# OthmanB/TAMCMC-C-

Measured on AMD Instinct MI355X. Metric: MALA steps/sec (all chains) + achieved HBM GB/s, 64 chains × 1e5-bin spectrum, higher is better.
Workload: dtype f64; 1 GPU; C2: model_MS_Global_a1etaa3_HarveyLike (id 2), 21 modes l=0..2, 56 params, 100000 bins, 64 chains per GPU, trunc_c=20, logL + gradient over 44 variables, params resident in HBM; chains_total=64

## Files before the change

tamcmc-c-_amd/csrc/tamcmc_eval_body.h:

```cpp
#ifndef TAMCMC_EVAL_BODY_H
#define TAMCMC_EVAL_BODY_H
#include <hip/hip_runtime.h>
#include "tamcmc_dev.h"

#define TM_WAVES (TM_THREADS / 64)

typedef const __attribute__((address_space(4))) TmMult *TmMultK;
typedef const __attribute__((address_space(4))) TmCellRec *TmCellRecK;
typedef const __attribute__((address_space(4))) TmTileHdr *TmTileHdrK;
typedef const __attribute__((address_space(4))) TmNoise *TmNoiseK;
typedef const __attribute__((address_space(4))) int32_t *TmIdxK;
typedef const __attribute__((address_space(4))) TmActive *TmActiveK;

typedef int TmEntry __attribute__((ext_vector_type(4)));
__device__ __forceinline__ TmEntry tm_load_entry(TmActiveK p)
{
    return *reinterpret_cast<const __attribute__((address_space(4))) TmEntry *>(p);
}

__device__ __forceinline__ double tm_rcp(double x)
{
    double r = __builtin_amdgcn_rcp(x);
    double e = __builtin_fma(-x, r, 1.0);
    r = __builtin_fma(r, e, r);
    e = __builtin_fma(-x, r, 1.0);
    r = __builtin_fma(r, e, r);
    return r;
}

__device__ __forceinline__ double tm_rcp1(double x)
{
    double r = __builtin_amdgcn_rcp(x);
    const double e = __builtin_fma(-x, r, 1.0);
    return __builtin_fma(r, e, r);
}

template <int MASK>
__device__ __forceinline__ unsigned tm_xor_dw(unsigned v, int lane)
{
    if constexpr (MASK == 1) return __builtin_amdgcn_update_dpp(0u, v, 0xB1, 0xf, 0xf, false);
    else if constexpr (MASK == 2) return __builtin_amdgcn_update_dpp(0u, v, 0x4E, 0xf, 0xf, false);
    else if constexpr (MASK == 4) {
        const unsigned r = __builtin_amdgcn_update_dpp(0u, v, 0x104, 0xf, 0x5, false);
        return __builtin_amdgcn_update_dpp(r, v, 0x114, 0xf, 0xa, false);
    } else if constexpr (MASK == 8) return __builtin_amdgcn_update_dpp(0u, v, 0x128, 0xf, 0xf, false);
    else if constexpr (MASK == 16) {
        const auto r = __builtin_amdgcn_permlane16_swap(v, v, false, false);
        return (lane & 16) ? r[0] : r[1];
    } else {
        const auto r = __builtin_amdgcn_permlane32_swap(v, v, false, false);
        return (lane & 32) ? r[0] : r[1];
    }
}

template <int MASK>
__device__ __forceinline__ double tm_xor(double v, int lane)
{
    const unsigned long long b = __double_as_longlong(v);
    const unsigned lo = tm_xor_dw<MASK>((unsigned)b, lane), hi = tm_xor_dw<MASK>((unsigned)(b >> 32), lane);
    return __longlong_as_double(((unsigned long long)hi << 32) | lo);
}

template <int MASK>
__device__ __forceinline__ double tm_swap_add(double a, double b)
{
    static_assert(MASK == 16 || MASK == 32, "two-register swaps exist for 16 and 32 lanes");
    const unsigned long long ba = __double_as_longlong(a), bb = __double_as_longlong(b);
    unsigned r0l, r1l, r0h, r1h;
    if constexpr (MASK == 32) {
        const auto l = __builtin_amdgcn_permlane32_swap((unsigned)ba, (unsigned)bb, false, false);
        const auto h = __builtin_amdgcn_permlane32_swap((unsigned)(ba >> 32), (unsigned)(bb >> 32), false, false);
        r0l = l[0]; r1l = l[1]; r0h = h[0]; r1h = h[1];
    } else {
        const auto l = __builtin_amdgcn_permlane16_swap((unsigned)ba, (unsigned)bb, false, false);
        const auto h = __builtin_amdgcn_permlane16_swap((unsigned)(ba >> 32), (unsigned)(bb >> 32), false, false);
        r0l = l[0]; r1l = l[1]; r0h = h[0]; r1h = h[1];
    }
    const double r0 = __longlong_as_double(((unsigned long long)r0h << 32) | r0l);
    const double r1 = __longlong_as_double(((unsigned long long)r1h << 32) | r1l);
    return r0 + r1;
}

__device__ __forceinline__ double tm_wave_sum(double v)
{
    const int lane = threadIdx.x & 63;
    v += tm_xor<32>(v, lane);
    v += tm_xor<16>(v, lane);
    v += tm_xor<8>(v, lane);
    v += tm_xor<4>(v, lane);
    v += tm_xor<2>(v, lane);
    v += tm_xor<1>(v, lane);
    return v;
}

__device__ __forceinline__ double tm_wave_prod(double v)
{
    const int lane = threadIdx.x & 63;
    v *= tm_xor<32>(v, lane);
    v *= tm_xor<16>(v, lane);
    v *= tm_xor<8>(v, lane);
    v *= tm_xor<4>(v, lane);
    v *= tm_xor<2>(v, lane);
    v *= tm_xor<1>(v, lane);
    return v;
}


__device__ __forceinline__ double tm_poly(TmCellRecK tr, double z)
{
    double p = tr->bg[TM_PDEG];
#pragma unroll
    for (int j = TM_PDEG - 1; j >= 0; j--) p = __builtin_fma(p, z, tr->bg[j]);
    return p;
}

template <int N, int MASK>
struct TmBfly {
    static constexpr int NE = (N + 1) & ~1;
    static constexpr int H = NE / 2;
    __device__ static __forceinline__ void run(double (&v)[TM_GSLOTS], int lane)
    {
        if constexpr (N == 1) {
            v[0] += tm_xor<MASK>(v[0], lane);
        } else if constexpr (MASK >= 16) {
#pragma unroll
            for (int i = 0; i < H; i++) v[i] = tm_swap_add<MASK>(v[i], (i + H < N) ? v[i + H] : 0.0);
        } else {
            const bool hi = (lane & MASK) != 0;
#pragma unroll
            for (int i = 0; i < H; i++) {
                const double up = (i + H < N) ? v[i + H] : 0.0;
                const double send = hi ? v[i] : up;
                const double keep = hi ? up : v[i];
                v[i] = keep + tm_xor<MASK>(send, lane);
            }
        }
        if constexpr (MASK > 1) TmBfly<(N == 1 ? 1 : H), MASK / 2>::run(v, lane);
    }
    __device__ static __forceinline__ int slot_of(int lane, bool &valid)
    {
        if constexpr (N == 1) {
            return 0;
        } else {
            int sub = 0;
            if constexpr (MASK > 1) sub = TmBfly<H, MASK / 2>::slot_of(lane, valid);
            const int idx = sub + (((lane & MASK) != 0) ? H : 0);
            if (idx >= N) valid = false;
            return idx;
        }
    }
};

template <int NC>
__device__ __forceinline__ double tm_mult_value(double x2, const double (&nu2)[NC], const double (&hq)[NC], double g2,
                                                double (&d)[NC], double (&r)[NC])
{
    double E[NC], P[NC];
#pragma unroll
    for (int m = 0; m < NC; m++) {
        d[m] = x2 - nu2[m];
        E[m] = __builtin_fma(d[m], d[m], g2);
    }
    P[0] = E[0];
#pragma unroll
    for (int m = 1; m < NC; m++) P[m] = P[m - 1] * E[m];
    double inv = tm_rcp1(P[NC - 1]);
    double s = 0.0;
#pragma unroll
    for (int m = NC - 1; m >= 1; m--) {
        r[m] = inv * P[m - 1];
        inv = inv * E[m];
    }
    r[0] = inv;
#pragma unroll
    for (int m = 0; m < NC; m++) s = __builtin_fma(hq[m], r[m], s);
    return s;
}

template <int NC>
__device__ __forceinline__ double tm_mult_sum(double x2, const double (&nu2)[NC], const double (&hq)[NC], double g2)
{
    double d = x2 - nu2[0];
    double Q = __builtin_fma(d, d, g2);
    double N = hq[0];
#pragma unroll
    for (int m = 1; m < NC; m++) {
        d = x2 - nu2[m];
        const double E = __builtin_fma(d, d, g2);
        N = __builtin_fma(hq[m], Q, N * E);
        Q = Q * E;
    }
    return N * tm_rcp(Q);
}

template <int NC, int KG, bool ASYM>
__device__ __forceinline__ void tm_accum_mult(TmMultK sm, const double (&x2)[KG], const int (&bi)[KG], double (&acc)[KG], const bool edge)
{
    double nu2[NC], hq[NC];
#pragma unroll
    for (int m = 0; m < NC; m++) { nu2[m] = sm->nu2[m]; hq[m] = sm->hq[m]; }
    const double g2 = sm->g2;
    const double aAh = ASYM ? 0.5 * sm->aA : 0.0, aB = ASYM ? sm->aB : 1.0, c2 = ASYM ? sm->c2 : 0.0;
    double s[KG];
#pragma unroll
    for (int k = 0; k < KG; k++) {
        s[k] = tm_mult_sum<NC>(x2[k], nu2, hq, g2);
        if (ASYM) {
            const double a = __builtin_fma(x2[k], aAh, aB);
            s[k] = s[k] * __builtin_fma(a, a, c2);
        }
    }
    if (edge) {
        const int imin = sm->imin, imax = sm->imax;
#pragma unroll
        for (int k = 0; k < KG; k++) {
            const bool inside = (bi[k] >= imin) && (bi[k] < imax);
            s[k] = inside ? s[k] : 0.0;
        }
    }
#pragma unroll
    for (int k = 0; k < KG; k++) acc[k] += s[k];
}

template <int KG>
__device__ __forceinline__ void tm_accum_dispatch(TmMultK sm, const int shape, const double (&x2)[KG], const int (&bi)[KG], double (&acc)[KG], const bool edge)
{
    switch (shape) {
    case 1: tm_accum_mult<1, KG, false>(sm, x2, bi, acc, edge); break;
    case 3: tm_accum_mult<3, KG, false>(sm, x2, bi, acc, edge); break;
    case 5: tm_accum_mult<5, KG, false>(sm, x2, bi, acc, edge); break;
    case 7: tm_accum_mult<7, KG, false>(sm, x2, bi, acc, edge); break;
    case 256 + 1: tm_accum_mult<1, KG, true>(sm, x2, bi, acc, edge); break;
    case 256 + 3: tm_accum_mult<3, KG, true>(sm, x2, bi, acc, edge); break;
    case 256 + 5: tm_accum_mult<5, KG, true>(sm, x2, bi, acc, edge); break;
    default: tm_accum_mult<7, KG, true>(sm, x2, bi, acc, edge); break;
    }
}

template <int NC> struct TmGradSlots {
    static constexpr int L = (NC - 1) / 2;
    static constexpr int A0 = NC, C = NC + L + 1, ASYM0 = NC + L + 2;
    __device__ static constexpr int count(bool asym) { return asym ? ASYM0 + 3 : ASYM0; }
};
template <int NC> __device__ __forceinline__ int tm_grad_store_slot(int v)
{
    using SL = TmGradSlots<NC>;
    return (v < NC) ? v : (v < SL::C) ? 7 + (v - NC) : (v == SL::C) ? 11 : 21 + (v - SL::ASYM0);
}

template <int NC, bool ASYM>
__device__ __forceinline__ void tm_grad_bin(const double (&nu2)[NC], const double (&hq)[NC], double g2, double aAh, double aB, double c2,
                                            const double x2, const double wk, double (&g)[TM_GSLOTS])
{
    using SL = TmGradSlots<NC>;
    double d[NC], r[NC];
    const double Sv = tm_mult_value<NC>(x2, nu2, hq, g2, d, r);
    double wA = wk;
    if (ASYM) {
        const double a = __builtin_fma(x2, aAh, aB);
        wA = wk * __builtin_fma(a, a, c2);
        const double ws = wk * Sv;
        g[SL::ASYM0 + 0] += ws;
        g[SL::ASYM0 + 1] = __builtin_fma(ws, a, g[SL::ASYM0 + 1]);
        g[SL::ASYM0 + 2] = __builtin_fma(ws * a, 0.5 * x2, g[SL::ASYM0 + 2]);
    }
#pragma unroll
    for (int m = 0; m < NC; m++) {
        const double t1 = wA * r[m];
        const double t2 = t1 * r[m];
        const int am = (m >= SL::L) ? m - SL::L : SL::L - m;
        g[SL::A0 + am] += t1;
        g[m] = __builtin_fma(t2, d[m], g[m]);
        g[SL::C] = __builtin_fma(hq[m], t2, g[SL::C]);
    }
}

template <int NC, bool ASYM>
__device__ __forceinline__ void tm_grad_unit(const double (&nu2)[NC], const double (&hq)[NC], double g2, double aAh, double aB, double c2,
                                             int imin, int imax, const double *__restrict__ gx, const double *wq, int i0, int Nx,
                                             const bool edge, double (&g)[TM_GSLOTS])
{
#pragma unroll
    for (int k = 0; k < 2; k++) {
        double x2, wk;
        if (edge) {
            const int i = i0 + k * TM_THREADS;
            const bool inside = (i >= imin) && (i < imax) && (i < Nx);
            x2 = gx[i < Nx ? i : Nx - 1];
            wk = inside ? wq[k * TM_THREADS] : 0.0;
        } else {
            x2 = gx[i0 + k * TM_THREADS];
            wk = wq[k * TM_THREADS];
        }
        tm_grad_bin<NC, ASYM>(nu2, hq, g2, aAh, aB, c2, x2, wk, g);
    }
}

template <int NC, bool ASYM>
__device__ __forceinline__ void tm_grad_unit_held(const double (&nu2)[NC], const double (&hq)[NC], double g2, double aAh, double aB, double c2,
                                                  int imin, int imax, const double (&xv)[2], const double (&wv)[2], int lo, int tid, int Nx,
                                                  const bool edge, double (&g)[TM_GSLOTS])
{
    double wk[2] = {wv[0], wv[1]};
    if (edge) {
#pragma unroll
        for (int k = 0; k < 2; k++) {
            const int i = lo + tid + k * TM_THREADS;
            const bool inside = (i >= imin) && (i < imax) && (i < Nx);
            wk[k] = inside ? wk[k] : 0.0;
        }
        asm volatile("" : "+v"(wk[0]), "+v"(wk[1]));
    }
#pragma unroll
    for (int k = 0; k < 2; k++) tm_grad_bin<NC, ASYM>(nu2, hq, g2, aAh, aB, c2, xv[k], wk[k], g);
}

__device__ __forceinline__ void tm_grad_fetch(const double *__restrict__ gx, const double *s_w, int u, int u0, int Nx, int tid,
                                              double (&xv)[2], double (&wv)[2])
{
    const int lo = u << TM_UNIT_SHIFT;
    if (lo + TM_UNIT_BINS <= Nx) {
        typedef const __attribute__((address_space(1))) double *TmGlobalD;
        TmGlobalD xb = (TmGlobalD)(gx + lo);
        asm volatile("" : "+s"(xb));
#pragma unroll
        for (int k = 0; k < 2; k++) xv[k] = xb[(unsigned)(tid + k * TM_THREADS)];
    } else {
#pragma unroll
        for (int k = 0; k < 2; k++) { const int i = lo + tid + k * TM_THREADS; xv[k] = gx[i < Nx ? i : Nx - 1]; }
        asm volatile("");
    }
    const double *wq = s_w + (u - u0) * TM_UNIT_BINS + tid;
#pragma unroll
    for (int k = 0; k < 2; k++) wv[k] = wq[k * TM_THREADS];
}

template <int NC, bool ASYM, bool AHEAD_>
__device__ __forceinline__ void tm_grad_mult(TmMultK sm, const double *__restrict__ gx, const double *s_w,
                                             int u0, int u1, int Nx, int tid, int lane, double *s_red_row)
{
    constexpr bool AHEAD = AHEAD_ && NC < 7;
    constexpr int V = TmGradSlots<NC>::count(ASYM);
    double g[TM_GSLOTS];
    double nu2[NC], hq[NC];
#pragma unroll
    for (int m = 0; m < NC; m++) { nu2[m] = sm->nu2[m]; hq[m] = sm->hq[m]; }
    const double g2 = sm->g2;
    const int imin = sm->imin, imax = sm->imax;
    const double aAh = ASYM ? 0.5 * sm->aA : 0.0, aB = ASYM ? sm->aB : 1.0, c2 = ASYM ? sm->c2 : 0.0;
#pragma unroll
    for (int s = 0; s < TM_GSLOTS; s++) g[s] = 0.0;
    if constexpr (AHEAD) {
        int ua = imin >> TM_UNIT_SHIFT, ub = (imax + TM_UNIT_BINS - 1) >> TM_UNIT_SHIFT;
        ua = ua > u0 ? ua : u0;
        ub = ub < u1 ? ub : u1;
        if (ua < ub) {
            double xc[2], wc[2];
            tm_grad_fetch(gx, s_w, ua, u0, Nx, tid, xc, wc);
            asm volatile("" : "+v"(xc[0]), "+v"(xc[1]), "+v"(wc[0]), "+v"(wc[1]));
            double xd[2], wd[2];
#pragma unroll 1
            for (int u = ua;;) {
                tm_grad_fetch(gx, s_w, u + 1 < ub ? u + 1 : u, u0, Nx, tid, xd, wd);
                {
                    const int lo = u << TM_UNIT_SHIFT, hi = lo + TM_UNIT_BINS;
                    tm_grad_unit_held<NC, ASYM>(nu2, hq, g2, aAh, aB, c2, imin, imax, xc, wc, lo, tid, Nx, !(lo >= imin && hi <= imax && hi <= Nx), g);
                }
                if (++u >= ub) break;
                tm_grad_fetch(gx, s_w, u + 1 < ub ? u + 1 : u, u0, Nx, tid, xc, wc);
                {
                    const int lo = u << TM_UNIT_SHIFT, hi = lo + TM_UNIT_BINS;
                    tm_grad_unit_held<NC, ASYM>(nu2, hq, g2, aAh, aB, c2, imin, imax, xd, wd, lo, tid, Nx, !(lo >= imin && hi <= imax && hi <= Nx), g);
                }
                if (++u >= ub) break;
            }
        }
    } else {
#pragma unroll 1
        for (int u = u0; u < u1; u++) {
            const int lo = u << TM_UNIT_SHIFT, hi = lo + TM_UNIT_BINS;
            if (hi <= imin || lo >= imax) continue;
            const double *wq = s_w + (u - u0) * TM_UNIT_BINS + tid;
            tm_grad_unit<NC, ASYM>(nu2, hq, g2, aAh, aB, c2, imin, imax, gx, wq, lo + tid, Nx, !(lo >= imin && hi <= imax && hi <= Nx), g);
        }
    }
#if defined(TM_ABLATE) && (TM_ABLATE & 1)
    if (lane == 0) s_red_row[0] = g[0] + g[1] + g[2];
    return;
#endif
    if constexpr (AHEAD) asm volatile("" : "+v"(lane));
    TmBfly<V, 32>::run(g, lane);
    constexpr int NSPLIT = (V > 16) ? 5 : (V > 8) ? 4 : (V > 4) ? 3 : (V > 2) ? 2 : 1;
    const int lowmask = (64 >> NSPLIT) - 1;
    bool valid = true;
    const int slot = TmBfly<V, 32>::slot_of(lane, valid);
    if ((lane & lowmask) == 0 && valid) {
        s_red_row[tm_grad_store_slot<NC>(slot)] = g[0];
    }
}

#ifndef TM_LB_FWD
#define TM_LB_FWD 4
#endif
#ifndef TM_LB_GRAD
#define TM_LB_GRAD 4
#endif
#ifndef TM_LOOKAHEAD
#define TM_LOOKAHEAD 1
#endif
#ifdef TM_TRACE
__device__ unsigned long long *g_tm_trace = nullptr;
#define TM_STAMP(slot) do { if (threadIdx.x == 0 && g_tm_trace) g_tm_trace[((size_t)blockIdx.y * gridDim.x + blockIdx.x) * 4 + (slot)] = wall_clock64(); } while (0)
#else
#define TM_STAMP(slot) do { } while (0)
#endif

#pragma clang fp contract(off)
__device__ __forceinline__ double tm_add_plain(double a, double b) { return a + b; }
#pragma clang fp contract(fast)

template <int N> struct TmInt { static constexpr int value = N; };
template <bool B> struct TmBool { static constexpr bool value = B; };

enum TmCellKind { TM_CK_POLY = 0, TM_CK_EXP = 1, TM_CK_NONE = 2, TM_CK_ANY = 3 };

template <bool GRAD, bool GEN = true>
__device__ __forceinline__ void tm_eval_body(const TmEvalArgs &a, const int chain, const int tile, double *s_w)
{
    const int like = GEN ? a.likelihood_case : 0;
    const int tid = threadIdx.x;
    const int lane = tid & 63, wave = tid >> 6;
    TmNoiseK sn = (TmNoiseK)(a.noise + chain);

#if defined(TM_ABLATE) && (TM_ABLATE & 16)
    if (a.Nx > 0) return;
#endif
    __shared__ double s_red[2][TM_WAVES][TM_GSLOTS];

    const size_t spec_off = (a.spec != nullptr) ? (size_t)((TmIdxK)a.spec)[chain] * (size_t)a.Nx : 0;
    const double *__restrict__ yp = a.y + spec_off;
    const double *__restrict__ isp = a.isig2 + spec_off;
    const TmMult *__restrict__ gm = a.mult + (size_t)chain * a.n_mult;
    TmTileHdrK th = (TmTileHdrK)(a.thdr + (size_t)chain * a.tiles + tile);
    const int u0 = th->u0;
    int u1 = th->u1;
    if (u1 - u0 > (GRAD ? TM_TILE_MAXU : TM_TILE_MAXU_L)) u1 = u0 + (GRAD ? TM_TILE_MAXU : TM_TILE_MAXU_L);
    const int nact = th->nact;
    TmCellRecK cells = (TmCellRecK)(a.cell + (size_t)chain * a.cells);
    TmActiveK tix = (TmActiveK)(a.tidx + ((size_t)chain * a.tiles + tile) * (a.n_mult > 0 ? a.n_mult : 1));
    const int nh = sn->nh;
    const bool has_gauss = GEN && sn->has_gauss != 0;
    const double N0 = sn->N0;
    const int row = (GEN && a.row_of_chain != nullptr) ? a.row_of_chain[chain] : -1;
    const double *__restrict__ xb = a.x2;
    const double *__restrict__ lb = a.lx;

#if defined(TM_ABLATE) && (TM_ABLATE & 32)
    if (nact >= 0 && N0 == N0) { if (tid == 0 && !GRAD) a.part[((size_t)chain * a.tiles + tile) * 4] = (double)(nh + row + u0 + (has_gauss ? 1 : 0)); return; }
#endif
    double S1 = 0.0;
    double P = 1.0;
    int esum = 0;
    int sgn = 0;
    double gn_[GRAD ? TM_GSLOTS : 1];
#pragma unroll
    for (int s_ = 0; s_ < (GRAD ? TM_GSLOTS : 1); s_++) gn_[s_] = 0.0;
    const double wscale = GRAD ? a.wt[2 * chain + 1] : 0.0;

    auto group = [&](auto kg_c, auto full_c, auto kind_c, const int u, TmCellRecK tr) __attribute__((always_inline)) {
        constexpr int KG = decltype(kg_c)::value;
        constexpr bool FULL = decltype(full_c)::value;
        constexpr int CK = decltype(kind_c)::value & 7;
        constexpr bool COLD = (decltype(kind_c)::value & 8) != 0;
        constexpr bool RT = CK == TM_CK_ANY;
        const bool HARVEY = RT ? nh > 0 : CK != TM_CK_NONE;
        const bool NPOLY = RT ? (nh > 0 && tr->npoly != 0) : CK == TM_CK_POLY;
        const int lo = u << TM_UNIT_SHIFT, hi = lo + KG * TM_THREADS;
        int nhx = nh;
        if constexpr (COLD) asm volatile("" : "+s"(nhx));
        double x2[KG], acc[KG];
        int bi[KG];
#pragma unroll
        for (int k = 0; k < KG; k++) {
            const int i = lo + k * TM_THREADS + tid;
            if (FULL) {
                bi[k] = i;
                x2[k] = xb[(unsigned)i];
            } else {
                const bool valid = i < a.Nx;
                bi[k] = valid ? i : -1;
                x2[k] = a.x2[valid ? i : a.Nx - 1];
            }
            acc[k] = 0.0;
        }
        constexpr bool EARLY = FULL && !GRAD && !COLD;
        double lxe[EARLY ? KG : 1], ye[EARLY ? KG : 1];
        if constexpr (EARLY) {
#pragma unroll
            for (int k = 0; k < KG; k++) { lxe[k] = HARVEY ? lb[(unsigned)bi[k]] : 0.0; ye[k] = yp[(unsigned)bi[k]]; }
        }
        if constexpr (GRAD) {
            for (int jj = 0; jj < nact; jj++) {
                const int idx = tix[jj].idx, imin = tix[jj].imin, imax = tix[jj].imax, shape = tix[jj].shape;
                if (hi <= imin || lo >= imax) continue;
                tm_accum_dispatch<KG>((TmMultK)(gm + idx), shape, x2, bi, acc, !(FULL && lo >= imin && hi <= imax));
            }
        } else if (nact > 0) {
            TmEntry e = tm_load_entry(tix);
            asm volatile("" :: "s"(e.x));
            for (int jj = 0; jj < nact; jj++) {
                const TmEntry en = tm_load_entry(tix + (jj + 1 < nact ? jj + 1 : jj));
                const int idx = e.x, imin = e.y, imax = e.z, shape = e.w;
                if (!(hi <= imin || lo >= imax))
                    tm_accum_dispatch<KG>((TmMultK)(gm + idx), shape, x2, bi, acc, !(FULL && lo >= imin && hi <= imax));
                e = en;
            }
        }

        constexpr int KH = GRAD ? 2 : KG;
#pragma unroll
        for (int h0 = 0; h0 < KG; h0 += KH) {
        double hu[TM_MAXH][GRAD ? KH : 1], harg[GRAD ? KH : 1];
        const bool n0_done = NPOLY;
        if (HARVEY) {
            double dl[KH];
#pragma unroll
            for (int k = 0; k < KH; k++) {
#if defined(TM_ABLATE) && (TM_ABLATE & 128)
                dl[k] = tr->lxc + 1e-9 * x2[h0 + k];
#else
                dl[k] = EARLY ? lxe[h0 + k] : FULL ? lb[(unsigned)bi[h0 + k]] : a.lx[bi[h0 + k] >= 0 ? bi[h0 + k] : a.Nx - 1];
#endif
                if constexpr (GRAD) harg[k] = dl[k];
            }
            if (NPOLY) {
                const double lxc = tr->lxc;
#pragma unroll
                for (int k = 0; k < KH; k++) { dl[k] -= lxc; acc[h0 + k] += tm_poly(tr, dl[k]); if constexpr (GRAD) harg[k] = dl[k]; }
            } else {
#pragma unroll
                for (int h = 0; h < TM_MAXH; h++) {
                    if (h < nhx) {
                        const double Hh = sn->H[h], ph = sn->p[h], lth = sn->lt[h];
#pragma unroll
                        for (int k = 0; k < KH; k++) {
                            const double t = exp(ph * (lth + dl[k]));
                            const double uu = 1.0 / (t + 1.0);
                            acc[h0 + k] += Hh * uu;
                            if constexpr (GRAD) hu[h][k] = uu;
                        }
                    }
                }
            }
        }
        if (has_gauss) {
            const double gA = sn->gA, gnu0 = sn->gnu0, gs2 = sn->gs2;
#pragma unroll
            for (int k = 0; k < KH; k++) {
                const double dd = 0.5 * x2[h0 + k] - gnu0;
                acc[h0 + k] = gA * exp((-0.5 * (dd * dd)) / gs2) + acc[h0 + k];
            }
        }
        if (!n0_done) {
#pragma unroll
            for (int k = 0; k < KH; k++) acc[h0 + k] += N0;
        }
        if (row >= 0) {
#pragma unroll
            for (int k = 0; k < KH; k++)
                if (FULL || bi[h0 + k] >= 0) a.model_out[(size_t)row * a.Nx + (size_t)(lo + (h0 + k) * TM_THREADS + tid)] = acc[h0 + k];
        }

        double wreg[GRAD ? KH : 1];
        if (like == 0) {
#pragma unroll
            for (int k = 0; k < KH; k++) {
                double wv = 0.0;
                if (FULL || bi[h0 + k] >= 0) {
                    const double M = acc[h0 + k];
                    const double yv = EARLY ? ye[h0 + k] : FULL ? yp[(unsigned)bi[h0 + k]] : yp[bi[h0 + k]];
                    sgn |= __double2hiint(M);
                    const double rM = tm_rcp(M);
                    S1 = __builtin_fma(yv, rM, S1);
                    int e;
                    P *= frexp(M, &e);
                    esum += e;
                    wv = wscale * (yv * rM * rM - rM);
                }
                if constexpr (GRAD) wreg[k] = wv;
            }
            {
                int e;
                P = frexp(P, &e);
                esum += e;
            }
        } else {
#pragma unroll
            for (int k = 0; k < KH; k++) {
                double wv = 0.0;
                if (FULL || bi[h0 + k] >= 0) {
                    const int i = lo + (h0 + k) * TM_THREADS + tid;
                    const double dd = yp[i] - acc[h0 + k];
                    const double is2 = isp[i];
                    S1 = __builtin_fma(dd * dd, is2, S1);
                    wv = wscale * dd * is2;
                }
                if constexpr (GRAD) wreg[k] = wv;
            }
        }
        if constexpr (GRAD) {
#pragma unroll
            for (int k = 0; k < KH; k++) {
                const double wk = wreg[k];
                s_w[((u - u0) * 2 + h0 + k) * TM_THREADS + tid] = wk;
                gn_[3 * TM_MAXH] = tm_add_plain(gn_[3 * TM_MAXH], wk);
#if defined(TM_ABLATE) && (TM_ABLATE & 512)
                if (false) {
#else
                if (NPOLY) {
#endif
                    double q = wk;
#pragma unroll
                    for (int j = 0; j < TM_HSER - 1; j++) { gn_[j] = __builtin_fma(harg[k], q, gn_[j]); q *= harg[k]; }
                } else if (HARVEY) {
#pragma unroll
                    for (int h = 0; h < TM_MAXH; h++) {
                        if (h < nhx) {
                            const double wu = wk * hu[h][k];
                            const double tu2 = wu * (1.0 - hu[h][k]);
                            gn_[3 * h] = __builtin_fma(wk, hu[h][k], gn_[3 * h]);
                            gn_[3 * h + 1] = __builtin_fma(wu, 1.0 - hu[h][k], gn_[3 * h + 1]);
                            gn_[3 * h + 2] = __builtin_fma(tu2, sn->lt[h] + harg[k], gn_[3 * h + 2]);
                        }
                    }
                }
                if (has_gauss) {
                    const double dd = 0.5 * x2[h0 + k] - sn->gnu0;
                    const double we = wk * exp((-0.5 * (dd * dd)) / sn->gs2);
                    gn_[13] += we;
                    gn_[14] = __builtin_fma(we, dd, gn_[14]);
                    gn_[15] = __builtin_fma(we * dd, dd, gn_[15]);
                }
            }
        }
        if constexpr (GRAD) __builtin_amdgcn_sched_barrier(0);
        }
    };

    auto flush_noise = [&](const int part, auto cold_c) __attribute__((always_inline)) {
        if constexpr (GRAD) {
            int ln = lane, td = tid;
            if constexpr (decltype(cold_c)::value) asm volatile("" : "+v"(ln), "+v"(td));
            static_assert(TM_NSLOTS == 16, "butterfly below assumes 16 noise slots");
            TmBfly<TM_NSLOTS, 32>::run(gn_, ln);
            bool valid = true;
            const int slot = TmBfly<TM_NSLOTS, 32>::slot_of(ln, valid);
            double *red = s_red[1][wave];
            if ((ln & 3) == 0) red[slot] = gn_[0];
            __syncthreads();
            if (td < TM_NSLOTS) {
                double t = 0.0;
#pragma unroll
                for (int wv = 0; wv < TM_WAVES; wv++) t += s_red[1][wv][td];
                a.gnoise[(((size_t)chain * a.tiles + tile) * 2 + part) * TM_NSLOTS + td] = t;
            }
            __syncthreads();
#pragma unroll
            for (int s_ = 0; s_ < TM_GSLOTS; s_++) gn_[s_] = 0.0;
        }
    };

    {
        auto walk = [&](auto kind_c, int u, const int ue, TmCellRecK tr) __attribute__((always_inline)) {
            if ((u & 1) && u < ue && ((u + 1) << TM_UNIT_SHIFT) <= a.Nx) { group(TmInt<2>(), TmBool<true>(), kind_c, u, tr); u += 1; }
#pragma unroll 1
            for (; u + 2 <= ue && ((u + 2) << TM_UNIT_SHIFT) <= a.Nx; u += 2) group(TmInt<4>(), TmBool<true>(), kind_c, u, tr);
#pragma unroll 1
            for (; u < ue; u += 1) {
                if (((u + 1) << TM_UNIT_SHIFT) <= a.Nx) group(TmInt<2>(), TmBool<true>(), kind_c, u, tr);
                else                                    group(TmInt<2>(), TmBool<false>(), kind_c, u, tr);
            }
        };
        auto walk_single = [&](auto kind_c, int u, const int ue, TmCellRecK tr) __attribute__((always_inline)) {
#pragma unroll 1
            for (; u < ue; u += 1) {
                if (((u + 1) << TM_UNIT_SHIFT) <= a.Nx) group(TmInt<2>(), TmBool<true>(), kind_c, u, tr);
                else                                    group(TmInt<2>(), TmBool<false>(), kind_c, u, tr);
            }
        };
        const int cell0 = u0 >> TM_CELL_SHIFT;
        int ce = cell0;
        int u = u0;
#if defined(TM_ABLATE) && (TM_ABLATE & 256)
        u = u1;
#endif
        if constexpr (GEN) {
            int cur_cell = cell0;
            auto cell_of = [&](const int uu) __attribute__((always_inline)) {
                const int c = uu >> TM_CELL_SHIFT;
                if (GRAD && c != cur_cell) { flush_noise(0, TmBool<false>()); cur_cell = c; }
                return cells + c;
            };
            if ((u & 1) && u < u1 && ((u + 1) << TM_UNIT_SHIFT) <= a.Nx) { TmCellRecK tr = cell_of(u); group(TmInt<2>(), TmBool<true>(), TmInt<TM_CK_ANY>(), u, tr); u += 1; }
#pragma unroll 1
            for (; u + 2 <= u1 && ((u + 2) << TM_UNIT_SHIFT) <= a.Nx; u += 2) { TmCellRecK tr = cell_of(u); group(TmInt<4>(), TmBool<true>(), TmInt<TM_CK_ANY>(), u, tr); }
#pragma unroll 1
            for (; u < u1; u += 1) {
                TmCellRecK tr = cell_of(u);
                if (((u + 1) << TM_UNIT_SHIFT) <= a.Nx) group(TmInt<2>(), TmBool<true>(), TmInt<TM_CK_ANY>(), u, tr);
                else                                    group(TmInt<2>(), TmBool<false>(), TmInt<TM_CK_ANY>(), u, tr);
            }
            ce = cur_cell + 1;
        } else {
#pragma unroll 1
            for (; u < u1; ce++) {
                TmCellRecK tr = cells + ce;
                if (nh <= 0 || tr->npoly == 0) break;
                if (GRAD && ce != cell0) flush_noise(0, TmBool<false>());
                const int cend = (ce + 1) << TM_CELL_SHIFT;
                const int ue = cend < u1 ? cend : u1;
                walk(TmInt<TM_CK_POLY>(), u, ue, tr);
                u = ue;
            }
#pragma unroll 1
            for (; u < u1; ce++) {
                TmCellRecK tr = cells + ce;
                if (GRAD && ce != cell0) flush_noise(0, TmBool<true>());
                const int cend = (ce + 1) << TM_CELL_SHIFT;
                const int ue = cend < u1 ? cend : u1;
                if (nh <= 0)             walk_single(TmInt<8 + TM_CK_NONE>(), u, ue, tr);
                else if (tr->npoly != 0) walk_single(TmInt<8 + TM_CK_POLY>(), u, ue, tr);
                else                     walk_single(TmInt<8 + TM_CK_EXP>(), u, ue, tr);
                u = ue;
            }
        }
        if (GRAD) flush_noise(ce > cell0 + 1 ? 1 : 0, TmBool<false>());
    }
    TM_STAMP(1);
    double Pm = 1.0, Pe = 0.0;
    if (like == 0) {
        int e;
        Pm = frexp(tm_wave_prod(P), &e);
        Pe = tm_wave_sum((double)esum) + (double)e;
        if (__builtin_amdgcn_ballot_w64(sgn < 0) != 0) Pm = __builtin_nan("");
    }
    S1 = tm_wave_sum(S1);
    if (lane == 0) { s_red[0][wave][0] = S1; s_red[0][wave][1] = Pm; s_red[0][wave][2] = Pe; }
    __syncthreads();
    if constexpr (GRAD) {
        if (tid == 0) {
            double t1 = 0.0, tm = 1.0, te = 0.0;
#pragma unroll
            for (int wv = 0; wv < TM_WAVES; wv++) { t1 += s_red[0][wv][0]; tm *= s_red[0][wv][1]; te += s_red[0][wv][2]; }
            double *out = a.part + ((size_t)chain * a.tiles + tile) * 4;
            out[0] = t1;
            out[1] = tm;
            out[2] = te;
        }
    } else if (wave == 0) {
        int last = 0;
        double *pp = a.part + (size_t)chain * a.tiles * 4;
        if (lane == 0) {
            double t1 = 0.0, tm = 1.0, te = 0.0;
#pragma unroll
            for (int wv = 0; wv < TM_WAVES; wv++) { t1 += s_red[0][wv][0]; tm *= s_red[0][wv][1]; te += s_red[0][wv][2]; }
#if defined(TM_ABLATE) && (TM_ABLATE & 4)
            pp[4 * tile] = t1; pp[4 * tile + 1] = tm; pp[4 * tile + 2] = te;
#else
            if (a.tiles == 1) {
                pp[0] = t1; pp[1] = tm; pp[2] = te;
                const double t2 = (like == 0) ? tm_tile_logsum(tm, te) : 0.0;
                double f = (like == 0) ? -a.like_p * (t1 + t2) : -t1;
                f = f / a.wt[2 * chain];
                int st = a.noise[chain].status;
                if (st != 0) f = __builtin_nan("");
                else if (!(f == f)) st = 1;
                a.logL[chain] = f;
                if (a.status) a.status[chain] = st;
            } else {
            __hip_atomic_store(pp + 4 * tile, t1, __ATOMIC_RELAXED, __HIP_MEMORY_SCOPE_AGENT);
            __hip_atomic_store(pp + 4 * tile + 1, tm, __ATOMIC_RELAXED, __HIP_MEMORY_SCOPE_AGENT);
            __hip_atomic_store(pp + 4 * tile + 2, te, __ATOMIC_RELAXED, __HIP_MEMORY_SCOPE_AGENT);
            asm volatile("s_waitcnt vmcnt(0)" ::: "memory");
            const int prev = __hip_atomic_fetch_add(a.ticket + chain, 1, __ATOMIC_RELAXED, __HIP_MEMORY_SCOPE_AGENT);
            last = (prev == a.tiles - 1) ? 1 : 0;
            }
#endif
        }
        last = __shfl(last, 0, 64);
        if (last) {
            double s1 = 0.0, s2 = 0.0;
            for (int t = lane; t < a.tiles; t += 64) {
                s1 += __hip_atomic_load(pp + 4 * t, __ATOMIC_RELAXED, __HIP_MEMORY_SCOPE_AGENT);
                if (like == 0)
                    s2 += tm_tile_logsum(__hip_atomic_load(pp + 4 * t + 1, __ATOMIC_RELAXED, __HIP_MEMORY_SCOPE_AGENT),
                                         __hip_atomic_load(pp + 4 * t + 2, __ATOMIC_RELAXED, __HIP_MEMORY_SCOPE_AGENT));
            }
            s1 = tm_wave_sum(s1);
            s2 = tm_wave_sum(s2);
            if (lane == 0) {
                double f = (like == 0) ? -a.like_p * (s1 + s2) : -s1;
                f = f / a.wt[2 * chain];
                int st = a.noise[chain].status;
                if (st != 0) f = __builtin_nan("");
                else if (!(f == f)) st = 1;
                a.logL[chain] = f;
                if (a.status) a.status[chain] = st;
                __hip_atomic_store(a.ticket + chain, 0, __ATOMIC_RELAXED, __HIP_MEMORY_SCOPE_AGENT);
            }
        }
    }

    TM_STAMP(2);
#ifdef TM_TRACE
    if (threadIdx.x == 0 && g_tm_trace) {
        unsigned hw;
        asm volatile("s_getreg_b32 %0, hwreg(HW_REG_HW_ID)" : "=s"(hw));
        unsigned xcc;
        asm volatile("s_getreg_b32 %0, hwreg(HW_REG_XCC_ID)" : "=s"(xcc));
        g_tm_trace[((size_t)blockIdx.y * gridDim.x + blockIdx.x) * 4 + 3] = ((unsigned long long)xcc << 32) | hw;
    }
#endif
    if constexpr (GRAD) {
        constexpr bool AHEAD = !GEN && TM_LOOKAHEAD != 0;
        __syncthreads();
#if defined(TM_ABLATE) && (TM_ABLATE & 2)
        for (int jj = 0; jj < 0; jj++) {
#else
        for (int jj = 0; jj < nact; jj++) {
#endif
            const int idx = tix[jj].idx, shape = tix[jj].shape;
            TmMultK sm = (TmMultK)(gm + idx);
            const int nc = shape & 255;
            double *red = s_red[(jj + 1) & 1][wave];
            if (lane == 0) {
                const int Lm = (nc - 1) >> 1;
                for (int am = Lm + 1; am <= 3; am++) red[7 + am] = 0.0;
                if (shape < 256) { red[21] = 0.0; red[22] = 0.0; red[23] = 0.0; }
            }
            switch (shape) {
            case 1: tm_grad_mult<1, false, AHEAD>(sm, a.x2, s_w, u0, u1, a.Nx, tid, lane, red); break;
            case 3: tm_grad_mult<3, false, AHEAD>(sm, a.x2, s_w, u0, u1, a.Nx, tid, lane, red); break;
            case 5: tm_grad_mult<5, false, AHEAD>(sm, a.x2, s_w, u0, u1, a.Nx, tid, lane, red); break;
            case 7: tm_grad_mult<7, false, AHEAD>(sm, a.x2, s_w, u0, u1, a.Nx, tid, lane, red); break;
            case 256 + 1: tm_grad_mult<1, true, AHEAD>(sm, a.x2, s_w, u0, u1, a.Nx, tid, lane, red); break;
            case 256 + 3: tm_grad_mult<3, true, AHEAD>(sm, a.x2, s_w, u0, u1, a.Nx, tid, lane, red); break;
            case 256 + 5: tm_grad_mult<5, true, AHEAD>(sm, a.x2, s_w, u0, u1, a.Nx, tid, lane, red); break;
            default: tm_grad_mult<7, true, AHEAD>(sm, a.x2, s_w, u0, u1, a.Nx, tid, lane, red); break;
            }
#if defined(TM_ABLATE) && (TM_ABLATE & 64)
            if (tid < TM_GSLOTS) a.gmult[(((size_t)chain * a.tiles + tile) * a.n_mult + idx) * TM_GSLOTS + tid] = red[tid];
#else
            __syncthreads();
            if (tid < TM_GSLOTS) {
                double t = 0.0;
                if (tid < nc || (tid >= 7 && tid < 12) || tid >= 21) {
#pragma unroll
                    for (int wv = 0; wv < TM_WAVES; wv++) t += s_red[(jj + 1) & 1][wv][tid];
                }
                a.gmult[(((size_t)chain * a.tiles + tile) * a.n_mult + idx) * TM_GSLOTS + tid] = t;
            }
#endif
        }
        TM_STAMP(2);
    }
}

#endif
```

Measured before the change: 714,300 chain-steps/s (model+logL+grad).

## Batch per-mode gradient reductions into shared rows and flush once per group

Gradient partial sums from the noise flushes, the logL partials and up to six mode multiplets now go into a per-wave shared row buffer. They are reduced and written to global memory in one flush per group of six multiplets, replacing a block barrier and a reduction after every multiplet and noise flush. The lookahead loop also peels off the partial last unit so the main fetch path can skip its bounds check. This cuts the number of __syncthreads in the gradient tile but adds shared-memory footprint, which may lower occupancy. The gnoise write for part 2 is now conditional, which relies on it not being needed in other cases.

```diff
diff --git a/tamcmc-c-_amd/csrc/tamcmc_eval_body.h b/tamcmc-c-_amd/csrc/tamcmc_eval_body.h
--- a/tamcmc-c-_amd/csrc/tamcmc_eval_body.h
+++ b/tamcmc-c-_amd/csrc/tamcmc_eval_body.h
@@ -4,6 +4,21 @@
 #include "tamcmc_dev.h"
 
 #define TM_WAVES (TM_THREADS / 64)
+
+#define TM_ROW_K 6
+#define TM_ROWS (3 + TM_ROW_K)
+static_assert(TM_ROWS * TM_GSLOTS <= TM_THREADS, "the flush takes one (row, slot) per thread");
+#ifndef TM_TILE_BARRIERS
+#define TM_TILE_BARRIERS 0
+#endif
+#ifndef TM_TAIL_APART
+#define TM_TAIL_APART 1
+#endif
+#if TM_TILE_BARRIERS
+#define TM_TILE_SYNC() __syncthreads()
+#else
+#define TM_TILE_SYNC() do { } while (0)
+#endif
 
 typedef const __attribute__((address_space(4))) TmMult *TmMultK;
 typedef const __attribute__((address_space(4))) TmCellRec *TmCellRecK;
@@ -315,11 +330,12 @@
     for (int k = 0; k < 2; k++) tm_grad_bin<NC, ASYM>(nu2, hq, g2, aAh, aB, c2, xv[k], wk[k], g);
 }
 
+template <bool WHOLE>
 __device__ __forceinline__ void tm_grad_fetch(const double *__restrict__ gx, const double *s_w, int u, int u0, int Nx, int tid,
                                               double (&xv)[2], double (&wv)[2])
 {
     const int lo = u << TM_UNIT_SHIFT;
-    if (lo + TM_UNIT_BINS <= Nx) {
+    if (WHOLE || lo + TM_UNIT_BINS <= Nx) {
         typedef const __attribute__((address_space(1))) double *TmGlobalD;
         TmGlobalD xb = (TmGlobalD)(gx + lo);
         asm volatile("" : "+s"(xb));
@@ -354,20 +370,24 @@
         int ua = imin >> TM_UNIT_SHIFT, ub = (imax + TM_UNIT_BINS - 1) >> TM_UNIT_SHIFT;
         ua = ua > u0 ? ua : u0;
         ub = ub < u1 ? ub : u1;
+        constexpr bool APART = TM_TAIL_APART != 0;
+        const int uw = Nx >> TM_UNIT_SHIFT;
+        const bool tail = APART && ub > uw && ua <= uw;
+        if (APART && ub > uw) ub = uw;
         if (ua < ub) {
             double xc[2], wc[2];
-            tm_grad_fetch(gx, s_w, ua, u0, Nx, tid, xc, wc);
+            tm_grad_fetch<APART>(gx, s_w, ua, u0, Nx, tid, xc, wc);
             asm volatile("" : "+v"(xc[0]), "+v"(xc[1]), "+v"(wc[0]), "+v"(wc[1]));
             double xd[2], wd[2];
 #pragma unroll 1
             for (int u = ua;;) {
-                tm_grad_fetch(gx, s_w, u + 1 < ub ? u + 1 : u, u0, Nx, tid, xd, wd);
+                tm_grad_fetch<APART>(gx, s_w, u + 1 < ub ? u + 1 : u, u0, Nx, tid, xd, wd);
                 {
                     const int lo = u << TM_UNIT_SHIFT, hi = lo + TM_UNIT_BINS;
                     tm_grad_unit_held<NC, ASYM>(nu2, hq, g2, aAh, aB, c2, imin, imax, xc, wc, lo, tid, Nx, !(lo >= imin && hi <= imax && hi <= Nx), g);
                 }
                 if (++u >= ub) break;
-                tm_grad_fetch(gx, s_w, u + 1 < ub ? u + 1 : u, u0, Nx, tid, xc, wc);
+                tm_grad_fetch<APART>(gx, s_w, u + 1 < ub ? u + 1 : u, u0, Nx, tid, xc, wc);
                 {
                     const int lo = u << TM_UNIT_SHIFT, hi = lo + TM_UNIT_BINS;
                     tm_grad_unit_held<NC, ASYM>(nu2, hq, g2, aAh, aB, c2, imin, imax, xd, wd, lo, tid, Nx, !(lo >= imin && hi <= imax && hi <= Nx), g);
@@ -375,6 +395,7 @@
                 if (++u >= ub) break;
             }
         }
+        if (tail) tm_grad_unit<NC, ASYM>(nu2, hq, g2, aAh, aB, c2, imin, imax, gx, s_w + (uw - u0) * TM_UNIT_BINS + tid, (uw << TM_UNIT_SHIFT) + tid, Nx, true, g);
     } else {
 #pragma unroll 1
         for (int u = u0; u < u1; u++) {
@@ -436,6 +457,7 @@
     if (a.Nx > 0) return;
 #endif
     __shared__ double s_red[2][TM_WAVES][TM_GSLOTS];
+    __shared__ double s_rows[TM_WAVES][TM_ROWS][TM_GSLOTS];
 
     const size_t spec_off = (a.spec != nullptr) ? (size_t)((TmIdxK)a.spec)[chain] * (size_t)a.Nx : 0;
     const double *__restrict__ yp = a.y + spec_off;
@@ -649,22 +671,16 @@
 
     auto flush_noise = [&](const int part, auto cold_c) __attribute__((always_inline)) {
         if constexpr (GRAD) {
-            int ln = lane, td = tid;
-            if constexpr (decltype(cold_c)::value) asm volatile("" : "+v"(ln), "+v"(td));
+            int ln = lane;
+            if constexpr (decltype(cold_c)::value) asm volatile("" : "+v"(ln));
             static_assert(TM_NSLOTS == 16, "butterfly below assumes 16 noise slots");
             TmBfly<TM_NSLOTS, 32>::run(gn_, ln);
             bool valid = true;
             const int slot = TmBfly<TM_NSLOTS, 32>::slot_of(ln, valid);
-            double *red = s_red[1][wave];
+            double *red = s_rows[wave][1 + part];
             if ((ln & 3) == 0) red[slot] = gn_[0];
-            __syncthreads();
-            if (td < TM_NSLOTS) {
-                double t = 0.0;
-#pragma unroll
-                for (int wv = 0; wv < TM_WAVES; wv++) t += s_red[1][wv][td];
-                a.gnoise[(((size_t)chain * a.tiles + tile) * 2 + part) * TM_NSLOTS + td] = t;
-            }
-            __syncthreads();
+            TM_TILE_SYNC();
+            TM_TILE_SYNC();
 #pragma unroll
             for (int s_ = 0; s_ < TM_GSLOTS; s_++) gn_[s_] = 0.0;
         }
@@ -745,18 +761,13 @@
         if (__builtin_amdgcn_ballot_w64(sgn < 0) != 0) Pm = __builtin_nan("");
     }
     S1 = tm_wave_sum(S1);
-    if (lane == 0) { s_red[0][wave][0] = S1; s_red[0][wave][1] = Pm; s_red[0][wave][2] = Pe; }
-    __syncthreads();
+    if constexpr (!GRAD) {
+        if (lane == 0) { s_red[0][wave][0] = S1; s_red[0][wave][1] = Pm; s_red[0][wave][2] = Pe; }
+        __syncthreads();
+    }
     if constexpr (GRAD) {
-        if (tid == 0) {
-            double t1 = 0.0, tm = 1.0, te = 0.0;
-#pragma unroll
-            for (int wv = 0; wv < TM_WAVES; wv++) { t1 += s_red[0][wv][0]; tm *= s_red[0][wv][1]; te += s_red[0][wv][2]; }
-            double *out = a.part + ((size_t)chain * a.tiles + tile) * 4;
-            out[0] = t1;
-            out[1] = tm;
-            out[2] = te;
-        }
+        if (lane == 0) { s_rows[wave][0][0] = S1; s_rows[wave][0][1] = Pm; s_rows[wave][0][2] = Pe; }
+        TM_TILE_SYNC();
     } else if (wave == 0) {
         int last = 0;
         double *pp = a.part + (size_t)chain * a.tiles * 4;
@@ -823,44 +834,67 @@
 #endif
     if constexpr (GRAD) {
         constexpr bool AHEAD = !GEN && TM_LOOKAHEAD != 0;
-        __syncthreads();
+        TM_TILE_SYNC();
 #if defined(TM_ABLATE) && (TM_ABLATE & 2)
-        for (int jj = 0; jj < 0; jj++) {
+        const int nrun = 0;
 #else
-        for (int jj = 0; jj < nact; jj++) {
-#endif
-            const int idx = tix[jj].idx, shape = tix[jj].shape;
-            TmMultK sm = (TmMultK)(gm + idx);
-            const int nc = shape & 255;
-            double *red = s_red[(jj + 1) & 1][wave];
-            if (lane == 0) {
-                const int Lm = (nc - 1) >> 1;
-                for (int am = Lm + 1; am <= 3; am++) red[7 + am] = 0.0;
-                if (shape < 256) { red[21] = 0.0; red[22] = 0.0; red[23] = 0.0; }
-            }
-            switch (shape) {
-            case 1: tm_grad_mult<1, false, AHEAD>(sm, a.x2, s_w, u0, u1, a.Nx, tid, lane, red); break;
-            case 3: tm_grad_mult<3, false, AHEAD>(sm, a.x2, s_w, u0, u1, a.Nx, tid, lane, red); break;
-            case 5: tm_grad_mult<5, false, AHEAD>(sm, a.x2, s_w, u0, u1, a.Nx, tid, lane, red); break;
-            case 7: tm_grad_mult<7, false, AHEAD>(sm, a.x2, s_w, u0, u1, a.Nx, tid, lane, red); break;
-            case 256 + 1: tm_grad_mult<1, true, AHEAD>(sm, a.x2, s_w, u0, u1, a.Nx, tid, lane, red); break;
-            case 256 + 3: tm_grad_mult<3, true, AHEAD>(sm, a.x2, s_w, u0, u1, a.Nx, tid, lane, red); break;
-            case 256 + 5: tm_grad_mult<5, true, AHEAD>(sm, a.x2, s_w, u0, u1, a.Nx, tid, lane, red); break;
-            default: tm_grad_mult<7, true, AHEAD>(sm, a.x2, s_w, u0, u1, a.Nx, tid, lane, red); break;
-            }
-#if defined(TM_ABLATE) && (TM_ABLATE & 64)
-            if (tid < TM_GSLOTS) a.gmult[(((size_t)chain * a.tiles + tile) * a.n_mult + idx) * TM_GSLOTS + tid] = red[tid];
-#else
+        const int nrun = nact;
+#endif
+#pragma unroll 1
+        for (int base = 0;; base += TM_ROW_K) {
+            const int nrow = nrun - base < TM_ROW_K ? nrun - base : TM_ROW_K;
+            const bool last = base + TM_ROW_K >= nrun;
+#pragma unroll 1
+            for (int j = 0; j < nrow; j++) {
+                const int jj = base + j;
+                const int idx = tix[jj].idx, shape = tix[jj].shape;
+                TmMultK sm = (TmMultK)(gm + idx);
+                double *red = s_rows[wave][3 + j];
+                switch (shape) {
+                case 1: tm_grad_mult<1, false, AHEAD>(sm, a.x2, s_w, u0, u1, a.Nx, tid, lane, red); break;
+                case 3: tm_grad_mult<3, false, AHEAD>(sm, a.x2, s_w, u0, u1, a.Nx, tid, lane, red); break;
+                case 5: tm_grad_mult<5, false, AHEAD>(sm, a.x2, s_w, u0, u1, a.Nx, tid, lane, red); break;
+                case 7: tm_grad_mult<7, false, AHEAD>(sm, a.x2, s_w, u0, u1, a.Nx, tid, lane, red); break;
+                case 256 + 1: tm_grad_mult<1, true, AHEAD>(sm, a.x2, s_w, u0, u1, a.Nx, tid, lane, red); break;
+                case 256 + 3: tm_grad_mult<3, true, AHEAD>(sm, a.x2, s_w, u0, u1, a.Nx, tid, lane, red); break;
+                case 256 + 5: tm_grad_mult<5, true, AHEAD>(sm, a.x2, s_w, u0, u1, a.Nx, tid, lane, red); break;
+                default: tm_grad_mult<7, true, AHEAD>(sm, a.x2, s_w, u0, u1, a.Nx, tid, lane, red); break;
+                }
+                TM_TILE_SYNC();
+            }
+#if !(defined(TM_ABLATE) && (TM_ABLATE & 64))
             __syncthreads();
-            if (tid < TM_GSLOTS) {
+#endif
+            const int r = tid / TM_GSLOTS, s = tid - r * TM_GSLOTS;
+            if (r >= 3 && r - 3 < nrow) {
+                const int idx = tix[base + r - 3].idx, shape = tix[base + r - 3].shape;
+                const int nc = shape & 255;
                 double t = 0.0;
-                if (tid < nc || (tid >= 7 && tid < 12) || tid >= 21) {
-#pragma unroll
-                    for (int wv = 0; wv < TM_WAVES; wv++) t += s_red[(jj + 1) & 1][wv][tid];
+                if (s < nc || (s >= 7 && s <= 7 + ((nc - 1) >> 1)) || s == 11 || (s >= 21 && shape >= 256)) {
+#pragma unroll
+                    for (int wv = 0; wv < TM_WAVES; wv++) t += s_rows[wv][r][s];
                 }
-                a.gmult[(((size_t)chain * a.tiles + tile) * a.n_mult + idx) * TM_GSLOTS + tid] = t;
-            }
-#endif
+                a.gmult[(((size_t)chain * a.tiles + tile) * a.n_mult + idx) * TM_GSLOTS + s] = t;
+            }
+            if (last) break;
+            __syncthreads();
+        }
+        {
+            const int r = tid / TM_GSLOTS, s = tid - r * TM_GSLOTS;
+            const size_t ct = (size_t)chain * a.tiles + tile;
+            if (r == 0) {
+                if (s < 3) {
+                    double t = (s == 1) ? 1.0 : 0.0;
+#pragma unroll
+                    for (int wv = 0; wv < TM_WAVES; wv++) { const double v = s_rows[wv][0][s]; t = (s == 1) ? t * v : t + v; }
+                    a.part[ct * 4 + s] = t;
+                }
+            } else if (r < 3 && s < TM_NSLOTS && (r == 1 || ((u1 - 1) >> TM_CELL_SHIFT) > (u0 >> TM_CELL_SHIFT))) {
+                double t = 0.0;
+#pragma unroll
+                for (int wv = 0; wv < TM_WAVES; wv++) t += s_rows[wv][r][s];
+                a.gnoise[(ct * 2 + (r - 1)) * TM_NSLOTS + s] = t;
+            }
         }
         TM_STAMP(2);
     }
```

Measured after the change: 726,900 chain-steps/s (model+logL+grad), median of 6. 1.8% higher.
